# arkworks-rs/snark

Hardware: NVIDIA H100
Metric: groth16_proofs_per_sec (higher is better)
Workload: dtype u32 limbs (255/381-bit modular integers)

## Files before the change

snark_b200/csrc/common.cuh:

```cuda
#pragma once
#include <cuda_runtime.h>

#include <cstdarg>
#include <cstdint>
#include <cstdio>
#include <map>
#include <mutex>
#include <string>
#include <vector>

#include "../../include/b200snark.h"
#include "curves.cuh"

namespace b2s {

struct NttPlan;
struct MsmDedupCache;

struct Ctx {
    int curve = 0;
    int device = 0;
    cudaStream_t stream = nullptr;
    cudaStream_t aux = nullptr;
    cudaEvent_t ev_tail = nullptr, ev_done = nullptr;
// ... 83 lines not shown
            p = nullptr;
            return fail(c, e == cudaErrorMemoryAllocation ? B2S_ERR_OOM : B2S_ERR_CUDA, "cudaMallocAsync(%zu): %s", n,
                        cudaGetErrorString(e));
        }
        return B2S_OK;
    }
    void release() {
        if (p && secret) cudaMemsetAsync(p, 0, bytes, ctx->stream);
        if (p) cudaFreeAsync(p, ctx->stream);
        p = nullptr;
        bytes = 0;
    }
    template <class T>
    T* as() const { return reinterpret_cast<T*>(p); }
};

struct InBuf {
    DevBuf own;
    const void* dptr = nullptr;
    int32_t bind(Ctx* c, const void* src, size_t bytes, int32_t mem) {
        if (mem == B2S_MEM_DEVICE) { dptr = src; return B2S_OK; }
        B2S_TRY(own.alloc(c, bytes));
        if (bytes) B2S_CUDA(c, cudaMemcpyAsync(own.p, src, bytes, cudaMemcpyHostToDevice, c->stream));
        dptr = own.p;
        return B2S_OK;
    }
    template <class T>
    const T* as() const { return reinterpret_cast<const T*>(dptr); }
};

#define B2S_SMEM_ATTR(ctx, kern, bytes) \
    B2S_CUDA(ctx, cudaFuncSetAttribute(kern, cudaFuncAttributeMaxDynamicSharedMemorySize, (int)(bytes)))

struct HostWipe {
    void* p;
    size_t n;
    ~HostWipe() {
        volatile unsigned char* q = reinterpret_cast<volatile unsigned char*>(p);
        for (size_t i = 0; i < n; i++) q[i] = 0;
    }
};

inline unsigned cdiv(uint64_t a, uint64_t b) { return (unsigned)((a + b - 1) / b); }

template <class F>
inline int32_t dispatch_curve(Ctx* c, F&& f) {
    switch (c->curve) {
        case B2S_CURVE_BLS12_381: return f(Bls12_381{});
        case B2S_CURVE_BN254: return f(Bn254{});
        case B2S_CURVE_BLS12_377: return f(Bls12_377{});
    }
    return fail(c, B2S_ERR_INVALID_ARG, "unknown curve id %d", c->curve);
}

struct Sizes {
    size_t fr, fq, g1, g2, g1x, g2x;
    size_t aff(int group) const { return group == 1 ? g1 : g2; }
    size_t xyzz(int group) const { return group == 1 ? g1x : g2x; }
    size_t enc(int group, bool compressed) const { return compressed ? aff(group) / 2 : aff(group); }
};
inline Sizes sizes(const Ctx* c) {
    Sizes s{};
    dispatch_curve(const_cast<Ctx*>(c), [&](auto curve) {
        using C = decltype(curve);
        using Fq = typename C::Fq;
        static_assert(sizeof(typename C::G1Affine) == 2 * sizeof(Fq) && sizeof(typename C::G2Affine) == 4 * sizeof(Fq) &&
                          sizeof(typename C::G1) == 4 * sizeof(Fq) && sizeof(typename C::G2) == 8 * sizeof(Fq),
                      "the ABI points are packed coordinates: 2, 4, 4 and 8 Fq");
        s = {sizeof(typename C::Fr), sizeof(Fq), sizeof(typename C::G1Affine), sizeof(typename C::G2Affine), sizeof(typename C::G1),
             sizeof(typename C::G2)};
        return (int32_t)B2S_OK;
    });
    return s;
}

int32_t ntt_run(Ctx* c, void* data_dev, uint32_t log_n, bool inverse, bool coset);
void ntt_free_plans(Ctx* c);
struct MsmPre { uint32_t c, nwin; uint32_t stride; };
int32_t msm_run(Ctx* c, int group, const void* bases_dev, const void* scalars_dev, uint64_t n, bool scalars_mont,
                void* out_xyzz_dev, void* wins_ext = nullptr, const MsmPre* pre = nullptr);
int32_t msm_run_batch(Ctx* c, int group, const void* bases_dev, const void* scalars_dev, uint64_t n, uint64_t stride, uint32_t K,
                      bool scalars_mont, void* out_xyzz_dev, const MsmPre* pre = nullptr);
uint64_t msm_batch_bytes(Ctx* c, int group, uint64_t n, const MsmPre* pre, uint64_t* max_k);
int32_t msm_precompute(Ctx* c, int group, const void* bases_dev, uint64_t n, void* table_dev, MsmPre* pre);
uint32_t msm_precompute_windows(Ctx* c, uint64_t n, uint32_t* c_out);
int32_t msm_join_tails(Ctx* c);
void msm_dedup_scope_begin(Ctx* c);
void msm_dedup_scope_end(Ctx* c);
int32_t scan_counts(Ctx* c, const uint32_t* counts, uint32_t n, uint32_t L, uint32_t* offsets, uint32_t* task_off);
int32_t fixed_base_run(Ctx* c, int group, const void* scalars_dev, uint64_t n, bool mont, void* out_dev);
int32_t group_sum_to_affine(Ctx* c, int group, const void* xyzz_dev, uint32_t count, void* out_affine_dev);

}
```

snark_b200/csrc/groth16.cu:

```cuda
#include "ec_team.cuh"
#include "r1cs.cuh"

namespace b2s {

template <class Curve>
__global__ void __launch_bounds__(128)
groth16_epilogue_g1_kernel(const Affine<typename Curve::Fq>* consts , const XYZZ<typename Curve::Fq>* sums ,
                           const typename Curve::Fr* rs, uint64_t rs_stride, Affine<typename Curve::Fq>* out_a, Affine<typename Curve::Fq>* out_c) {
    using Fq = typename Curve::Fq;
    using Fr = typename Curve::Fr;
    using P = XYZZ<Fq>;
    __shared__ P sh[3];
    __shared__ P table[3][16];
    const int role = threadIdx.x >> 5;
    const bool lead = (threadIdx.x & 31) == 0;
    sums += blockIdx.x;
    const uint32_t K = gridDim.x;
    rs += blockIdx.x * rs_stride;
    out_a += blockIdx.x;
    out_c += blockIdx.x;
    if (role == 0) {
        P a = sums[2 * K];
        a.add_affine(consts[0]);
        Fr s = rs[1].from_mont();
        P v = team_scalar_mul(a, s.v, Fr::N, table[0]);
        if (lead) sh[0] = v;
    } else if (role == 1) {
        P b = sums[3 * K];
        b.add_affine(consts[1]);
        Fr r = rs[0].from_mont();
        P v = team_scalar_mul(b, r.v, Fr::N, table[1]);
        if (lead) sh[1] = v;
    } else if (role == 2) {
        Fr rsp = (rs[0] * rs[1]).from_mont();
        P v = team_scalar_mul(P::from_affine(consts[2]), rsp.v, Fr::N, table[2]);
        if (lead) sh[2] = v;
    } else {
        P a = sums[2 * K];
        a.add_affine(consts[0]);
        if (lead) *out_a = a.to_affine();
    }
    __syncthreads();
    if (role == 0) {
        P c = sh[0];
        team_add(c, sh[1]);
        team_add(c, sh[2].neg());
        team_add(c, sums[K]);
        team_add(c, sums[0]);
        if (lead) *out_c = c.to_affine();
    }
}

template <class Curve>
__global__ void groth16_epilogue_g2_kernel(const Affine<typename Curve::Fq2>* consts ,
                                           const XYZZ<typename Curve::Fq2>* b2_sum, Affine<typename Curve::Fq2>* out_b) {
    if (threadIdx.x != 0) return;
    XYZZ<typename Curve::Fq2> acc = b2_sum[blockIdx.x];
    acc.add_affine(consts[0]);
    out_b[blockIdx.x] = acc.to_affine();
}

template <class F>
__global__ void sum_shards_kernel(const XYZZ<F>* partials, uint32_t n_shards, uint32_t stride, uint32_t count, XYZZ<F>* sums) {
    const uint32_t j = blockIdx.x * blockDim.x + threadIdx.x;
    if (j >= count) return;
    XYZZ<F> acc = XYZZ<F>::identity();
    for (uint32_t sidx = 0; sidx < n_shards; sidx++) acc.add(partials[sidx * stride + j]);
    sums[j] = acc;
}

int32_t pk_finish(Ctx* c, b2s_pk* pk) {
    const Sizes z = sizes(c);
    const uint64_t n_vars = pk->n_instance + pk->n_witness;
    const char* delta[3] = {nullptr, pk->consts_g1.as<char>() + 2 * z.g1, pk->consts_g2.as<char>() + z.g2};
    for (int w = 0; w < PK_QUERIES; w++) {
        PkQuery& q = pk->q[w];
        const PkQueryInfo& info = PK_QUERY[w];
        const size_t pt = z.aff(info.group);
        q.ext = (info.delta_at >= 0 && q.off + q.len == n_vars) ? 2 : 0;
        char* d = q.pts.as<char>() + q.len * pt;
        B2S_CUDA(c, cudaMemsetAsync(d, 0, 2 * pt, c->stream));
        if (q.ext) B2S_CUDA(c, cudaMemcpyAsync(d + info.delta_at * pt, delta[info.group], pt, cudaMemcpyDeviceToDevice, c->stream));
    }
    const PkQuery& h = pk->q[Q_H];
    {
        const char* env = getenv("B2S_PK_PRECOMP");
        const uint64_t min_n = getenv("B2S_PK_PRECOMP_MIN") ? strtoull(getenv("B2S_PK_PRECOMP_MIN"), nullptr, 10) : (1ull << 18);
        uint32_t cc = 0;
        const uint32_t nw = msm_precompute_windows(c, h.len, &cc);
        size_t free_b = 0, total_b = 0;
        cudaMemGetInfo(&free_b, &total_b);
        const uint64_t need = (uint64_t)nw * h.len * z.g1;
        if (!(env && env[0] == '0') && h.len >= min_n && (uint64_t)nw * h.len < (1ull << 31) && need * 4 < (uint64_t)free_b) {
            B2S_TRY(pk->h_table.alloc(c, need));
            B2S_TRY(msm_precompute(c, 1, h.pts.p, h.len, pk->h_table.p, &pk->h_pre));
        }
    }
    B2S_CUDA(c, cudaStreamSynchronize(c->stream));
    return B2S_OK;
}

int32_t pk_upload(Ctx* c, const b2s_pk_desc* d, int32_t mem, int32_t qap, b2s_pk** out) {
    const Sizes z = sizes(c);
    const uint64_t n_vars = d->n_instance + d->n_witness;
    struct { const void* pts; uint64_t off, len, bound; } src[PK_QUERIES] = {
        {d->a_query, d->a_off, d->a_len, n_vars},
        {d->b_g1_query, d->b1_off, d->b1_len, n_vars},
        {d->b_g2_query, d->b2_off, d->b2_len, n_vars},
        {d->h_query, d->h_off, d->h_len, d->domain_size},
        {d->l_query, d->l_off, d->l_len, d->n_witness}};
    for (const auto& s : src)
        if (s.off + s.len > s.bound) return fail(c, B2S_ERR_MALFORMED_VK, "pk: a query range exceeds the key dimensions");
    if (!d->alpha_g1 || !d->beta_g1 || !d->delta_g1 || !d->beta_g2 || !d->delta_g2)
        return fail(c, B2S_ERR_MALFORMED_VK, "pk: missing group constants");
    if (qap == B2S_QAP_CIRCOM && d->h_off == 0 && d->h_len + 1 == d->domain_size && d->a_len == n_vars && d->b1_len == n_vars &&
        d->b2_len == n_vars && d->l_len == d->n_witness)
        return fail(c, B2S_ERR_MALFORMED_VK, "pk: a full circom key has domain_size = %llu h_query points, not %llu (a libsnark key?)",
                    (unsigned long long)d->domain_size, (unsigned long long)d->h_len);
    b2s_pk* pk = new b2s_pk();
    pk->n_instance = d->n_instance; pk->n_witness = d->n_witness; pk->domain_size = d->domain_size; pk->qap = qap;
    for (int w = 0; w < PK_QUERIES; w++) { pk->q[w].off = src[w].off; pk->q[w].len = src[w].len; }
    const cudaMemcpyKind kind = mem == B2S_MEM_DEVICE ? cudaMemcpyDeviceToDevice : cudaMemcpyHostToDevice;
    auto body = [&]() -> int32_t {
        const size_t g1 = z.g1, g2 = z.g2;
        B2S_TRY(pk->consts_g1.alloc(c, 3 * g1));
        B2S_TRY(pk->consts_g2.alloc(c, 2 * g2));
        char* p1 = pk->consts_g1.as<char>();
        char* p2 = pk->consts_g2.as<char>();
        B2S_CUDA(c, cudaMemcpyAsync(p1, d->alpha_g1, g1, kind, c->stream));
        B2S_CUDA(c, cudaMemcpyAsync(p1 + g1, d->beta_g1, g1, kind, c->stream));
        B2S_CUDA(c, cudaMemcpyAsync(p1 + 2 * g1, d->delta_g1, g1, kind, c->stream));
        B2S_CUDA(c, cudaMemcpyAsync(p2, d->beta_g2, g2, kind, c->stream));
        B2S_CUDA(c, cudaMemcpyAsync(p2 + g2, d->delta_g2, g2, kind, c->stream));
        for (int w = 0; w < PK_QUERIES; w++) {
            const size_t pt = z.aff(PK_QUERY[w].group);
            B2S_TRY(pk->q[w].pts.alloc(c, (src[w].len + 2) * pt));
            if (src[w].len) B2S_CUDA(c, cudaMemcpyAsync(pk->q[w].pts.p, src[w].pts, src[w].len * pt, kind, c->stream));
        }
        return pk_finish(c, pk);
    };
    const int32_t st = body();
    if (st != B2S_OK) { delete pk; return st; }
    *out = pk;
    return B2S_OK;
}

struct ReplicatedH : HSource {
    DevBuf h;
    int32_t get(Ctx* c, const b2s_pk* pk, const b2s_r1cs* m, const void* z_dev, const void** h_for_shard) override {
        B2S_TRY(h.alloc(c, (size_t)32 << m->log_domain));
        B2S_TRY(witness_map_run(c, m, z_dev, h.p, pk->qap));
        *h_for_shard = h.as<char>() + pk->q[Q_H].off * 32;
        return B2S_OK;
    }
};

static int32_t pk_matches(Ctx* c, const b2s_pk* pk, const b2s_r1cs* m) {
    const uint64_t N = 1ull << m->log_domain;
    if (pk->n_instance != m->n_instance || pk->n_witness != m->n_witness || pk->domain_size != N)
        return fail(c, B2S_ERR_ASSIGNMENT_MISSING, "prove: key (%llu,%llu,%llu) does not match matrices (%llu,%llu,%llu)",
                    (unsigned long long)pk->n_instance, (unsigned long long)pk->n_witness, (unsigned long long)pk->domain_size,
                    (unsigned long long)m->n_instance, (unsigned long long)m->n_witness, (unsigned long long)N);
    return B2S_OK;
}

template <class Curve>
static int32_t shard_t(Ctx* c, const b2s_pk* pk, const b2s_r1cs* m, const void* z_inst, const void* z_wit, const void* z_dev,
                       const void* r_host, const void* s_host, void* g1_out, void* g2_out, HSource* hs) {
    using Fr = typename Curve::Fr;
    using P1 = XYZZ<typename Curve::Fq>;
    using P2 = XYZZ<typename Curve::Fq2>;
    B2S_TRY(pk_matches(c, pk, m));
    const uint64_t n_vars = m->n_instance + m->n_witness;
    DevBuf z, tails;
    ReplicatedH replicated;
    if (!hs) hs = &replicated;
    B2S_TRY(z.alloc(c, (n_vars + 2) * sizeof(Fr)));
    B2S_TRY(tails.alloc(c, 4 * 64 * sizeof(P1) + 64 * sizeof(P2)));
// ... 182 lines not shown
```

snark_b200/csrc/msm.cu:

```cuda
#include <algorithm>
#include <array>
#include <cstring>

#include "msm_affine.cuh"

namespace b2s {

__device__ __forceinline__ int32_t recode_digit(uint64_t v, uint32_t off, uint32_t& carry, uint32_t w, uint32_t c, uint32_t nwin) {
    uint32_t d = (uint32_t)((v >> off) & ((1u << c) - 1u)) + carry;
    carry = 0;
    if (w != nwin - 1 && d >= (1u << (c - 1))) {
        carry = 1;
        return (int32_t)d - (int32_t)(1u << c);
    }
    return (int32_t)d;
}

struct DigitIter {
    uint32_t k[8];
    uint32_t carry;
    __device__ __forceinline__ int32_t next(uint32_t w, uint32_t c, uint32_t nwin) {
        const uint32_t bit = w * c;
        const uint32_t word = bit >> 5, off = bit & 31;
        uint64_t v = 0;
// ... 376 lines not shown
            for (uint32_t p = (s + S - bb % S) % S; p < parts; p += S) {
                const uint32_t p0 = lo + p * SORT_SPLIT, p1 = min(hi, p0 + SORT_SPLIT);
                for (uint32_t i = p0 + threadIdx.x; i < p1; i += SORT_THREADS) atomicAdd(&hist[part_fine[i]], 1u);
                __syncthreads();
                for (uint32_t f = threadIdx.x; f < nf; f += SORT_THREADS) {
                    const uint32_t k = hist[f];
                    if (k) cur[f] = offsets[k0 + f] + atomicAdd(&cursor[k0 + f], k);
                    hist[f] = 0;
                }
                __syncthreads();
                for (uint32_t c0 = p0; c0 < p1; c0 += SORT_CHUNK) place_chunk(c0, min(SORT_CHUNK, p1 - c0), nf, part_val, part_fine, sorted, sv, sf, hist, start, cur);
            }
        }
        __syncthreads();
    }
}

struct HeavyPlan { uint32_t split, big, by_ordinal; };
static HeavyPlan heavy_plan(uint32_t G) { return G <= 64 ? HeavyPlan{256u, 512u, 1u} : HeavyPlan{16u, 256u, 0u}; }
static size_t heavy_tmp_slots(const HeavyPlan& hp, uint32_t G, uint64_t max_tasks) {
    return hp.by_ordinal ? (size_t)G * hp.split + 1 : (size_t)(max_tasks / hp.split) + hp.split + 1;
}

template <class F>
__global__ void __launch_bounds__(MSM_RED_THREADS)
msm_reduce_heavy_stage1_kernel(const uint32_t* __restrict__ heavy, const uint32_t* __restrict__ task_off, HeavyPlan hp,
                               const XYZZ<F>* __restrict__ partials, XYZZ<F>* __restrict__ tmp) {
    extern __shared__ uint4 smem_raw[];
    XYZZ<F>* smem = reinterpret_cast<XYZZ<F>*>(smem_raw);
    const uint32_t nitems = heavy[0] * hp.split;
    for (uint32_t it = blockIdx.x; it < nitems; it += gridDim.x) {
        const uint32_t h = it / hp.split, j = it % hp.split;
        const uint32_t g = heavy[1 + h];
        const uint32_t t0 = task_off[g], cnt = task_off[g + 1] - t0;
        if (cnt < hp.big) continue;
        const uint32_t lo = (uint32_t)((uint64_t)cnt * j / hp.split), hi = (uint32_t)((uint64_t)cnt * (j + 1) / hp.split);
        XYZZ<F> s = cta_sum(partials + t0 + lo, hi - lo, smem);
        if (threadIdx.x == 0) st_struct(tmp + (hp.by_ordinal ? h * hp.split : t0 / hp.split) + j, s);
        __syncthreads();
    }
}

template <class F>
__global__ void __launch_bounds__(MSM_RED_THREADS)
msm_reduce_heavy_kernel(const uint32_t* __restrict__ heavy, const uint32_t* __restrict__ task_off, const uint32_t* __restrict__ perm, HeavyPlan hp,
                        const XYZZ<F>* __restrict__ partials, const XYZZ<F>* __restrict__ tmp, XYZZ<F>* __restrict__ bucket_acc) {
    extern __shared__ uint4 smem_raw[];
    XYZZ<F>* smem = reinterpret_cast<XYZZ<F>*>(smem_raw);
    const uint32_t nheavy = heavy[0];
    for (uint32_t h = blockIdx.x; h < nheavy; h += gridDim.x) {
        const uint32_t rk = heavy[1 + h];
        const uint32_t g = perm ? perm[rk] : rk;
        const uint32_t t0 = task_off[rk], cnt = task_off[rk + 1] - t0;
        XYZZ<F> s = cnt < hp.big ? cta_sum(partials + t0, cnt, smem) : cta_sum(tmp + (hp.by_ordinal ? h * hp.split : t0 / hp.split), hp.split, smem);
        if (threadIdx.x == 0) st_struct(bucket_acc + g, s);
        __syncthreads();
    }
}

template <class F>
__global__ void __launch_bounds__(MSM_RED_THREADS)
group_sum_affine_kernel(const XYZZ<F>* __restrict__ pts, uint32_t count, Affine<F>* __restrict__ out) {
    extern __shared__ uint4 smem_raw[];
    XYZZ<F>* smem = reinterpret_cast<XYZZ<F>*>(smem_raw);
    XYZZ<F> s = cta_sum(pts, count, smem);
    if (threadIdx.x == 0) {
        Affine<F> a = s.to_affine();
        st_struct(out, a);
    }
}

int32_t msm_bucket_reduce_g2(Ctx* c, const void* bucket_acc, MsmShape sh, uint32_t seg, void* segs, uint32_t segs_per_win, void* wins) {
    return dispatch_curve(c, [&](auto curve) {
        using F = typename decltype(curve)::Fq2;
        return msm_bucket_reduce_launch<F>(c, "msm_bucket_segments_g2", "msm_window_sum_g2", bucket_acc, sh, seg, segs, segs_per_win, wins);
    });
}

static uint32_t env_u32(const char* name, uint32_t dflt) {
    const char* v = getenv(name);
    return v ? (uint32_t)strtoul(v, nullptr, 10) : dflt;
}

static MsmShape msm_shape(uint64_t n, uint32_t scalar_bits, size_t point_bytes, const MsmPre* pre = nullptr, uint32_t K = 1) {
    MsmShape sh{};
    if (pre) {
        sh.c = pre->c; sh.nwin = pre->nwin; sh.B = 1u << (pre->c - 1); sh.G = K * sh.B; sh.pre_stride = pre->stride;
        const uint64_t t_upper = (uint64_t)K * sh.nwin * n;
        sh.L = (uint32_t)std::max<uint64_t>(64, t_upper >> 18);
        sh.max_tasks = t_upper / sh.L + sh.G + 1;
        return sh;
    }
    auto nwin_of = [&](uint32_t c) {
        uint32_t nw = (scalar_bits + c - 1) / c;
        if (scalar_bits - (nw - 1) * c >= c) nw += 1;
        return nw;
    };
    uint32_t best_c = 5;
    double best = 1e300;
    for (uint32_t c = 5; c <= 20; c++) {
        const uint32_t nw = nwin_of(c);
        const double buckets = (double)nw * (double)(1u << (c - 1));
        if (buckets * (double)point_bytes > 4.0 * 1024 * 1024 * 1024) break;
        const double cost = (double)n * nw + buckets * 4.7;
        if (cost < best) { best = cost; best_c = c; }
    }
    uint32_t c = env_u32("B2S_MSM_C", best_c);
    if (c < 2) c = 2;
    if (c > 24) c = 24;
    sh.c = c;
    sh.nwin = nwin_of(c);
    sh.B = 1u << (c - 1);
    sh.G = K * sh.nwin * sh.B;
    const uint64_t t_upper = (uint64_t)K * sh.nwin * n;
    uint64_t L = t_upper >> 18;
    if (L < 64) L = 64;
    L = env_u32("B2S_MSM_L", (uint32_t)L);
    sh.L = (uint32_t)L;
    sh.max_tasks = t_upper / sh.L + sh.G + 1;
    return sh;
}

struct RoundPlan { uint32_t rounds, L; uint64_t max_tasks; };
template <class F>
static RoundPlan plan_rounds(Ctx* c, uint64_t T, uint32_t G, bool is_g1, uint32_t L_default) {
    RoundPlan rp{0, L_default, T / L_default + G + 1};
    uint32_t ba_auto = 0;
    const uint64_t per_bucket = G ? T / G : 0;
    while ((1ull << ba_auto) < per_bucket) ba_auto++;
    const double min_adds = is_g1 ? 6.0e6 : 2.5e6;
    uint32_t pays = 0;
    while (pays < 16 && (double)(T >> (pays + 1)) > min_adds) pays++;
    ba_auto = std::min(ba_auto, pays);
    rp.rounds = env_u32("B2S_MSM_AFFINE_ROUNDS", ba_auto);
    if (rp.rounds && !getenv("B2S_MSM_AFFINE_ROUNDS")) {
        const uint64_t t0 = std::min<uint64_t>(T, (T + G) / 2 + 1);
        const uint64_t need = t0 * (sizeof(Affine<F>) * 3 / 2 + sizeof(F)) + t0 / 4;
        size_t free_b = (size_t)c->total_mem, total_b = 0;
        uint64_t pool_held = 0;
        if (need * 3 > c->total_mem) {
            cudaMemGetInfo(&free_b, &total_b);
            cudaMemPool_t pool;
            if (cudaDeviceGetDefaultMemPool(&pool, c->device) == cudaSuccess) {
                uint64_t reserved = 0, used = 0;
                cudaMemPoolGetAttribute(pool, cudaMemPoolAttrReservedMemCurrent, &reserved);
                cudaMemPoolGetAttribute(pool, cudaMemPoolAttrUsedMemCurrent, &used);
                pool_held = reserved > used ? reserved - used : 0;
            }
        }
        if (need + ((uint64_t)2 << 30) > (uint64_t)free_b + pool_held) rp.rounds = 0;
    }
    if (rp.rounds && !getenv("B2S_MSM_L")) {
        uint64_t t_after = T;
        for (uint32_t r = 0; r < rp.rounds; r++) t_after = std::min<uint64_t>(t_after, (t_after + G) / 2 + 1);
        rp.L = (uint32_t)std::max<uint64_t>(16, t_after >> 18);
        rp.max_tasks = t_after / rp.L + G + 1;
    }
    return rp;
}

template <class Curve, class F>
static int32_t bucket_sums_t(Ctx* c, const Affine<F>* bases, const uint32_t* sorted, uint32_t* counts, uint32_t* offsets, uint64_t T, uint32_t G,
                             const RoundPlan& rp, XYZZ<F>* bucket_acc) {
    using Pt = XYZZ<F>;
    constexpr bool is_g1 = sizeof(F) == sizeof(typename Curve::Fq);
    MsmShape sh{};
    sh.G = G; sh.L = rp.L; sh.max_tasks = rp.max_tasks;
    const uint32_t ntiles = (G + SCAN_TILE - 1) / SCAN_TILE;
    const uint32_t* no_perm = nullptr;
    DevBuf tiles, tbuf, partials, heavy_tmp;
    B2S_TRY(tiles.alloc(c, (size_t)ntiles * sizeof(Scan3)));
    B2S_TRY(tbuf.alloc(c, ((size_t)2 * G + 3) * sizeof(uint32_t)));
    uint32_t* task_off = tbuf.as<uint32_t>();
    uint32_t* heavy = task_off + G + 1;
    B2S_TRY(partials.alloc(c, (size_t)sh.max_tasks * sizeof(Pt)));
    const HeavyPlan hp = heavy_plan(G);
    B2S_TRY(heavy_tmp.alloc(c, heavy_tmp_slots(hp, G, sh.max_tasks) * sizeof(Pt)));
    const void* acc_bases = bases;
    const uint32_t* acc_sorted = sorted;
    const uint32_t* acc_offsets = offsets;
    const uint32_t* acc_counts = counts;
    DevBuf ba_ints, ba_out[2], ba_prefix, ba_tot, ba_bits;
    if (rp.rounds) {
        B2S_TRY(ba_ints.alloc(c, ((size_t)4 * G + 2) * sizeof(uint32_t)));
        uint32_t* pp_cnt[2] = {ba_ints.as<uint32_t>(), ba_ints.as<uint32_t>() + 2 * G + 1};
        uint32_t* pp_off[2] = {pp_cnt[0] + G, pp_cnt[1] + G};
        const uint32_t* cnt_in = counts;
        uint64_t t_in = T;
        auto round_bound = [&](uint64_t tin) { return std::min<uint64_t>(tin, (tin + G) / 2 + 1); };
        const uint64_t out_bound0 = round_bound(t_in);
        const uint64_t words_bound0 = out_bound0 / 32 + 2;
        const uint64_t tot_bound = (words_bound0 / BA_KMIN + 2) * 32;
        const uint32_t rank_tiles0 = cdiv(words_bound0, BA_SCAN_TILE);
        B2S_TRY(ba_bits.alloc(c, (2 * words_bound0 + rank_tiles0 + 1) * sizeof(uint32_t)));
        uint32_t* bitmap = ba_bits.as<uint32_t>();
        uint32_t* wrank = bitmap + words_bound0;
        uint32_t* rtiles = wrank + words_bound0;
        B2S_TRY(ba_prefix.alloc(c, out_bound0 * sizeof(F)));
        B2S_TRY(ba_tot.alloc(c, 2 * tot_bound * sizeof(F)));
        const uint32_t target_units = 4u * 16u * (uint32_t)c->sm_count;
        DevBuf ba_ctr;
        B2S_TRY(ba_ctr.alloc(c, (size_t)2 * rp.rounds * sizeof(uint32_t)));
        B2S_CUDA(c, cudaMemsetAsync(ba_ctr.p, 0, (size_t)2 * rp.rounds * sizeof(uint32_t), c->stream));
        B2S_TRY(ba_out[1].alloc(c, out_bound0 * sizeof(Affine<F>)));
        if (rp.rounds > 1) B2S_TRY(ba_out[0].alloc(c, round_bound(out_bound0) * sizeof(Affine<F>)));
        const void* prev = nullptr;
        for (uint32_t r = 0; r < rp.rounds; r++) {
            const int nxt = (int)(r & 1u);
            uint32_t* cnt_out = pp_cnt[nxt];
            uint32_t* off_out = pp_off[nxt];
            const uint64_t out_bound = round_bound(t_in);
            const uint32_t n_words = (uint32_t)(out_bound / 32 + 2);
            const uint32_t rank_tiles = cdiv(n_words, BA_SCAN_TILE);
            B2S_LAUNCH(c, msm_ba_halve_kernel, cdiv(G, 256), 256, 0, cnt_in, G, cnt_out);
            B2S_LAUNCH(c, msm_scan_tiles_kernel, ntiles, SCAN_THREADS, 0, (const uint32_t*)cnt_out, no_perm, sh, tiles.as<Scan3>());
            B2S_LAUNCH(c, msm_scan_spine_kernel, 1, 1024, 0, tiles.as<Scan3>(), ntiles, sh, off_out, task_off, heavy);
            B2S_LAUNCH(c, msm_scan_apply_kernel, ntiles, SCAN_THREADS, 0, (const uint32_t*)cnt_out, no_perm, sh, tiles.as<Scan3>(), off_out, task_off, heavy);
            B2S_CUDA(c, cudaMemsetAsync(bitmap, 0, (size_t)n_words * sizeof(uint32_t), c->stream));
            B2S_LAUNCH(c, msm_ba_singles_kernel, cdiv(G, 256), 256, 0, cnt_in, (const uint32_t*)off_out, G, bitmap);
            B2S_LAUNCH(c, msm_ba_rank_tiles_kernel, rank_tiles, BA_SCAN_THREADS, 0, bitmap, n_words, rtiles);
            B2S_LAUNCH(c, msm_ba_rank_spine_kernel, 1, 1024, 0, rtiles, rank_tiles);
            B2S_LAUNCH(c, msm_ba_rank_apply_kernel, rank_tiles, BA_SCAN_THREADS, 0, bitmap, n_words, rtiles, wrank);
            BaRoundArgs ra{};
            ra.first = r == 0;
            ra.bases = bases; ra.sorted = sorted; ra.prev = prev;
            ra.bitmap = bitmap; ra.wrank = wrank; ra.t_out = off_out + G;
            ra.target_units = target_units;
            ra.unit_ctr = ba_ctr.as<uint32_t>() + 2 * r;
            ra.prefix = ba_prefix.p; ra.tot = ba_tot.p; ra.inv_scratch = ba_tot.as<F>() + tot_bound; ra.out = ba_out[nxt ^ 1].p;
            if (is_g1) B2S_TRY(msm_ba_round_g1(c, ra));
            else B2S_TRY(msm_ba_round_g2(c, ra));
            prev = ba_out[nxt ^ 1].p;
            t_in = out_bound;
            cnt_in = cnt_out;
        }
        acc_bases = prev;
        acc_sorted = nullptr;
        acc_offsets = pp_off[(rp.rounds - 1) & 1u];
        acc_counts = pp_cnt[(rp.rounds - 1) & 1u];
    } else {
        B2S_LAUNCH(c, msm_scan_tiles_kernel, ntiles, SCAN_THREADS, 0, counts, no_perm, sh, tiles.as<Scan3>());
        B2S_LAUNCH(c, msm_scan_spine_kernel, 1, 1024, 0, tiles.as<Scan3>(), ntiles, sh, offsets, task_off, heavy);
        B2S_LAUNCH(c, msm_scan_apply_kernel, ntiles, SCAN_THREADS, 0, counts, no_perm, sh, tiles.as<Scan3>(), offsets, task_off, heavy);
    }
    const uint32_t* perm = nullptr;
    DevBuf perm_buf;
    if (!rp.rounds && G >= 1024) {
        B2S_TRY(perm_buf.alloc(c, ((size_t)G + 2 * SIZE_BINS) * sizeof(uint32_t)));
        uint32_t* pm = perm_buf.as<uint32_t>();
        uint32_t* hist = pm + G;
        uint32_t* binoff = hist + SIZE_BINS;
        uint32_t* none = nullptr;
        B2S_CUDA(c, cudaMemsetAsync(hist, 0, SIZE_BINS * sizeof(uint32_t), c->stream));
        B2S_LAUNCH(c, msm_size_hist_kernel, cdiv(G, 256), 256, 0, acc_counts, G, hist);
        B2S_LAUNCH(c, msm_size_scan_kernel, 1, 1024, 0, hist, binoff);
        B2S_LAUNCH(c, msm_size_scatter_kernel, cdiv(G, 256), 256, 0, acc_counts, G, binoff, hist, pm);
        B2S_LAUNCH(c, msm_scan_tiles_kernel, ntiles, SCAN_THREADS, 0, acc_counts, (const uint32_t*)pm, sh, tiles.as<Scan3>());
        B2S_LAUNCH(c, msm_scan_spine_kernel, 1, 1024, 0, tiles.as<Scan3>(), ntiles, sh, none, task_off, heavy);
        B2S_LAUNCH(c, msm_scan_apply_kernel, ntiles, SCAN_THREADS, 0, acc_counts, (const uint32_t*)pm, sh, tiles.as<Scan3>(), none, task_off, heavy);
        perm = pm;
    }
    if (is_g1) B2S_TRY(msm_accumulate_g1(c, acc_bases, acc_sorted, acc_offsets, task_off, perm, sh, bucket_acc, partials.p));
    else B2S_TRY(msm_accumulate_g2(c, acc_bases, acc_sorted, acc_offsets, task_off, perm, sh, bucket_acc, partials.p));
    const size_t red_smem = (size_t)MSM_RED_THREADS * sizeof(Pt);
    B2S_SMEM_ATTR(c, msm_reduce_heavy_kernel<F>, red_smem);
    B2S_SMEM_ATTR(c, msm_reduce_heavy_stage1_kernel<F>, red_smem);
    B2S_LAUNCH(c, msm_reduce_heavy_stage1_kernel<F>, 4 * c->sm_count, MSM_RED_THREADS, red_smem, heavy, task_off, hp,
               partials.as<Pt>(), heavy_tmp.as<Pt>());
    B2S_LAUNCH(c, msm_reduce_heavy_kernel<F>, 2 * c->sm_count, MSM_RED_THREADS, red_smem, heavy, task_off, perm, hp,
               partials.as<Pt>(), heavy_tmp.as<Pt>(), bucket_acc);
    return B2S_OK;
}

template <class Curve, class F>
static int32_t msm_core_t(Ctx* c, const Affine<F>* bases, const typename Curve::Fr* scalars, const uint32_t* index_map, uint64_t n, bool mont,
                          XYZZ<F>* out, void* wins_ext, bool* used_aux = nullptr, const MsmPre* pre = nullptr, uint32_t K = 1, uint64_t stride = 0) {
    using Fr = typename Curve::Fr;
    using Pt = XYZZ<F>;
    constexpr bool is_g1 = sizeof(F) == sizeof(typename Curve::Fq);
    if (n == 0) {
        B2S_CUDA(c, cudaMemsetAsync(out, 0, K * sizeof(Pt), c->stream));
        return B2S_OK;
    }
    MsmShape sh = msm_shape(n, Curve::FrP::BITS, sizeof(Pt), pre, K);
    if ((uint64_t)K * sh.nwin * n >= (1ull << 32) || (uint64_t)K * sh.nwin * sh.B >= (1ull << 32))
        return fail(c, B2S_ERR_INVALID_ARG, "msm: vectors * n * windows exceeds 2^32");
    if (pre && (uint64_t)pre->nwin * pre->stride >= (1ull << 31)) return fail(c, B2S_ERR_INVALID_ARG, "msm: precomputed table exceeds 2^31 points");
    const RoundPlan rp = plan_rounds<F>(c, (uint64_t)K * sh.nwin * n, sh.G, is_g1, sh.L);
    sh.L = rp.L; sh.max_tasks = rp.max_tasks;
    const uint32_t MSM_SEG = sh.B >= (1u << 16) ? 32u : 16u;
    const uint32_t ntiles = (sh.G + SCAN_TILE - 1) / SCAN_TILE;
    DevBuf ibuf, sorted, bucket_acc, segs, wins, tiles;
    B2S_TRY(tiles.alloc(c, (size_t)ntiles * sizeof(Scan3)));
    const size_t ints = (size_t)5 * sh.G + 3;
    B2S_TRY(ibuf.alloc(c, ints * sizeof(uint32_t)));
    uint32_t* counts = ibuf.as<uint32_t>();
    uint32_t* cursor = counts + sh.G;
    uint32_t* offsets = cursor + sh.G;
    uint32_t* task_off = offsets + sh.G + 1;
    uint32_t* heavy = task_off + sh.G + 1;
    B2S_CUDA(c, cudaMemsetAsync(counts, 0, (size_t)2 * sh.G * sizeof(uint32_t), c->stream));
    const uint64_t T = (uint64_t)K * sh.nwin * n;
    B2S_TRY(sorted.alloc(c, (size_t)T * sizeof(uint32_t)));
    B2S_TRY(bucket_acc.alloc(c, (size_t)sh.G * sizeof(Pt)));
    B2S_CUDA(c, cudaMemsetAsync(bucket_acc.p, 0, (size_t)sh.G * sizeof(Pt), c->stream));
    const uint32_t segs_per_win = (sh.B + MSM_SEG - 1) / MSM_SEG;
    MsmShape sh_red = sh;
    sh_red.nwin = K * (pre ? 1u : sh.nwin);
    B2S_TRY(segs.alloc(c, (size_t)segs_per_win * sh_red.nwin * sizeof(Pt)));
    if (sh.nwin > 64 || K > 1) wins_ext = nullptr;
    if (!wins_ext) B2S_TRY(wins.alloc(c, (size_t)std::max(sh.nwin, sh_red.nwin) * sizeof(Pt)));
    Pt* wins_p = wins_ext ? reinterpret_cast<Pt*>(wins_ext) : wins.as<Pt>();

    B2S_LAUNCH(c, msm_count_kernel<Fr>, dim3(cdiv(n, 256), K), 256, 0, scalars, n, stride, mont, sh, counts);
    const uint32_t* no_perm = nullptr;
    B2S_LAUNCH(c, msm_scan_tiles_kernel, ntiles, SCAN_THREADS, 0, counts, no_perm, sh, tiles.as<Scan3>());
    B2S_LAUNCH(c, msm_scan_spine_kernel, 1, 1024, 0, tiles.as<Scan3>(), ntiles, sh, offsets, task_off, heavy);
    B2S_LAUNCH(c, msm_scan_apply_kernel, ntiles, SCAN_THREADS, 0, counts, no_perm, sh, tiles.as<Scan3>(), offsets, task_off, heavy);
    {
        const uint32_t fine_bits = sort_fine_bits(sh.c), nbins = sh.G >> fine_bits, nbw = sh.B >> fine_bits;
        DevBuf part;
        B2S_TRY(part.alloc(c, (size_t)T * (sizeof(uint32_t) + sizeof(uint16_t)) + (size_t)nbins * sizeof(uint32_t)));
        uint32_t* part_val = part.as<uint32_t>();
        uint32_t* bin_cursor = part_val + T;
        uint16_t* part_fine = reinterpret_cast<uint16_t*>(bin_cursor + nbins);
        B2S_CUDA(c, cudaMemsetAsync(bin_cursor, 0, (size_t)nbins * sizeof(uint32_t), c->stream));
        B2S_SMEM_ATTR(c, msm_partition_kernel<Fr>, partition_smem(nbw));
        B2S_SMEM_ATTR(c, msm_place_kernel, place_smem(fine_bits));
        B2S_LAUNCH(c, msm_partition_kernel<Fr>, dim3(cdiv(n, SORT_TILE), K), SORT_THREADS, partition_smem(nbw), scalars, index_map, n, stride, mont, sh,
                   fine_bits, (const uint32_t*)offsets, bin_cursor, part_val, part_fine);
        B2S_LAUNCH(c, msm_place_kernel, nbins + c->sm_count, SORT_THREADS, place_smem(fine_bits), (const uint32_t*)offsets, nbins, fine_bits,
                   (const uint32_t*)part_val, (const uint16_t*)part_fine, cursor, sorted.as<uint32_t>());
    }
    B2S_TRY((bucket_sums_t<Curve, F>(c, bases, sorted.as<uint32_t>(), counts, offsets, T, sh.G, rp, bucket_acc.as<Pt>())));
    if (is_g1) B2S_TRY(msm_bucket_reduce_g1(c, bucket_acc.p, sh_red, MSM_SEG, segs.p, segs_per_win, wins_p));
    else B2S_TRY(msm_bucket_reduce_g2(c, bucket_acc.p, sh_red, MSM_SEG, segs.p, segs_per_win, wins_p));
    if (!wins_ext) {
        B2S_TRY(msm_horner(c, c->stream, is_g1 ? 1 : 2, wins_p, sh_red, K, out));
    } else {
        B2S_CUDA(c, cudaEventRecord(c->ev_tail, c->stream));
        B2S_CUDA(c, cudaStreamWaitEvent(c->aux, c->ev_tail, 0));
        B2S_TRY(msm_horner(c, c->aux, is_g1 ? 1 : 2, wins_p, sh_red, K, out));
        c->aux_pending = true;
        if (used_aux) *used_aux = true;
    }
    return B2S_OK;
}

static constexpr uint32_t DEDUP_SAMPLES = 1024, DEDUP_MAX = 8;
struct DedupCand { uint32_t v[DEDUP_MAX][8]; uint32_t k; };

template <class Fr>
__global__ void msm_sample_kernel(const Fr* __restrict__ scalars, uint64_t n, uint64_t stride, Fr* __restrict__ out) {
    const uint32_t t = blockIdx.x * blockDim.x + threadIdx.x;
    if (t >= DEDUP_SAMPLES) return;
    const uint64_t i = (uint64_t)t * stride;
    if (i < n) st_struct(out + t, ld_struct(scalars + i));
}
template <class Fr>
__device__ __forceinline__ uint32_t dedup_gid(const Fr& s, const DedupCand& cd) {
    uint32_t nz = 0;
#pragma unroll
    for (int j = 0; j < 8; j++) nz |= s.v[j];
    if (nz == 0) return DEDUP_MAX + 1;
    for (uint32_t k = 0; k < cd.k; k++) {
        uint32_t d = 0;
#pragma unroll
        for (int j = 0; j < 8; j++) d |= s.v[j] ^ cd.v[k][j];
        if (d == 0) return k;
    }
    return DEDUP_MAX;
}
template <class Fr, int PASS>
// ... 196 lines not shown
        }
        B2S_LAUNCH_SN(c, ts, is_g1 ? "msm_tiny_products_g1" : "msm_tiny_products_g2", (msm_tiny_products_kernel<Curve, F>), count, 32, 0, bases,
                      (const uint32_t*)rest_idx.as<uint32_t>(), (const Fr*)rest_scal.as<Fr>(), (uint32_t)n_rest, (const Pt*)hsums, cd, mont, prods);
        B2S_LAUNCH_SN(c, ts, is_g1 ? "msm_tiny_sum_g1" : "msm_tiny_sum_g2", msm_tiny_sum_kernel<F>, 1, 32, 0, (const Pt*)prods, count, out);
        if (on_aux) c->aux_pending = true;
        return B2S_OK;
    }
    bool used_aux = false;
    B2S_TRY((msm_core_t<Curve, F>(c, bases, rest_scal.as<Fr>(), rest_idx.as<uint32_t>(), n_rest, mont, out, wins_ext, &used_aux, pre)));
    cudaStream_t fs = used_aux ? c->aux : c->stream;
    const size_t fin_smem = ((size_t)DEDUP_MAX * 16 + DEDUP_MAX) * sizeof(Pt);
    B2S_SMEM_ATTR(c, (msm_heavy_finish_kernel<Curve, F>), fin_smem);
    B2S_LAUNCH_SN(c, fs, is_g1 ? "msm_heavy_finish_g1" : "msm_heavy_finish_g2", (msm_heavy_finish_kernel<Curve, F>), 1, 32 * DEDUP_MAX, fin_smem,
                  (const Pt*)hsums, cd, mont, out);
    return B2S_OK;
}

int32_t scan_counts(Ctx* c, const uint32_t* counts, uint32_t n, uint32_t L, uint32_t* offsets, uint32_t* task_off) {
    MsmShape sh{};
    sh.G = n;
    sh.L = L;
    const uint32_t ntiles = (n + SCAN_TILE - 1) / SCAN_TILE;
    DevBuf tiles, heavy;
    B2S_TRY(tiles.alloc(c, (size_t)ntiles * sizeof(Scan3)));
    B2S_TRY(heavy.alloc(c, ((size_t)n + 1) * sizeof(uint32_t)));
    const uint32_t* no_perm = nullptr;
    B2S_LAUNCH(c, msm_scan_tiles_kernel, ntiles, SCAN_THREADS, 0, counts, no_perm, sh, tiles.as<Scan3>());
    B2S_LAUNCH(c, msm_scan_spine_kernel, 1, 1024, 0, tiles.as<Scan3>(), ntiles, sh, offsets, task_off, heavy.as<uint32_t>());
    B2S_LAUNCH(c, msm_scan_apply_kernel, ntiles, SCAN_THREADS, 0, counts, no_perm, sh, tiles.as<Scan3>(), offsets, task_off, heavy.as<uint32_t>());
    return B2S_OK;
}

int32_t msm_join_tails(Ctx* c) {
    if (!c->aux_pending) return B2S_OK;
    B2S_CUDA(c, cudaEventRecord(c->ev_done, c->aux));
    B2S_CUDA(c, cudaStreamWaitEvent(c->stream, c->ev_done, 0));
    c->aux_pending = false;
    return B2S_OK;
}

int32_t msm_run(Ctx* c, int group, const void* bases_dev, const void* scalars_dev, uint64_t n, bool scalars_mont,
                void* out_xyzz_dev, void* wins_ext, const MsmPre* pre) {
    return dispatch_curve(c, [&](auto curve) {
        using C = decltype(curve);
        if (group == 1) return msm_run_t<C, typename C::Fq>(c, bases_dev, scalars_dev, n, scalars_mont, out_xyzz_dev, wins_ext, pre);
        return msm_run_t<C, typename C::Fq2>(c, bases_dev, scalars_dev, n, scalars_mont, out_xyzz_dev, wins_ext, pre);
    });
}

int32_t msm_run_batch(Ctx* c, int group, const void* bases_dev, const void* scalars_dev, uint64_t n, uint64_t stride, uint32_t K,
                      bool scalars_mont, void* out_xyzz_dev, const MsmPre* pre) {
    if (n >= (1ull << 31)) return fail(c, B2S_ERR_INVALID_ARG, "msm: n = %llu exceeds 2^31 - 1", (unsigned long long)n);
    return dispatch_curve(c, [&](auto curve) {
        using C = decltype(curve);
        const auto* s = reinterpret_cast<const typename C::Fr*>(scalars_dev);
        if (group == 1) {
            using F = typename C::Fq;
            return msm_core_t<C, F>(c, reinterpret_cast<const Affine<F>*>(bases_dev), s, nullptr, n, scalars_mont, reinterpret_cast<XYZZ<F>*>(out_xyzz_dev),
                                    nullptr, nullptr, pre, K, stride);
        }
        using F = typename C::Fq2;
        return msm_core_t<C, F>(c, reinterpret_cast<const Affine<F>*>(bases_dev), s, nullptr, n, scalars_mont, reinterpret_cast<XYZZ<F>*>(out_xyzz_dev),
                                nullptr, nullptr, pre, K, stride);
    });
}

static uint32_t fr_bits(Ctx* c) {
    uint32_t bits = 0;
    dispatch_curve(c, [&](auto curve) { bits = decltype(curve)::FrP::BITS; return (int32_t)B2S_OK; });
    return bits;
}

uint64_t msm_batch_bytes(Ctx* c, int group, uint64_t n, const MsmPre* pre, uint64_t* max_k) {
    const Sizes z = sizes(c);
    const uint32_t bits = fr_bits(c);
    const size_t pt = z.xyzz(group);
    const MsmShape sh = msm_shape(std::max<uint64_t>(n, 1), bits, pt, pre);
    const uint64_t T = (uint64_t)sh.nwin * n, G = sh.G;
    *max_k = std::max<uint64_t>(1, std::min(((1ull << 32) - 1) / std::max<uint64_t>(T, 1), ((1ull << 32) - 1) / G));
    const uint64_t fe = z.aff(group) / 2;
    return G * (pt + 5 * sizeof(uint32_t)) + T * (sizeof(uint32_t) * 2 + sizeof(uint16_t)) + (T / 16 + G) * pt + T * (3 * fe + fe) / 2;
}

template <class F>
__global__ void __launch_bounds__(128) msm_precompute_kernel(const Affine<F>* __restrict__ bases, uint64_t n, uint32_t c, uint32_t nwin, Affine<F>* __restrict__ table) {
    const uint64_t i = (uint64_t)blockIdx.x * blockDim.x + threadIdx.x;
    if (i >= n) return;
    const Affine<F> p = ld_struct(bases + i);
    st_struct(table + i, p);
    XYZZ<F> acc = XYZZ<F>::from_affine(p);
    for (uint32_t w = 1; w < nwin; w++) {
        for (uint32_t k = 0; k < c; k++) acc = acc.dbl();
        const Affine<F> q = acc.to_affine();
        st_struct(table + (uint64_t)w * n + i, q);
        acc = XYZZ<F>::from_affine(q);
    }
}

uint32_t msm_precompute_windows(Ctx* c, uint64_t n, uint32_t* c_out) {
    (void)n;
    const uint32_t bits = fr_bits(c);
    const uint32_t cc = env_u32("B2S_MSM_PRE_C", 20);
    uint32_t nw = (bits + cc - 1) / cc;
    if (bits - (nw - 1) * cc >= cc) nw += 1;
    if (c_out) *c_out = cc;
    return nw;
}

int32_t msm_precompute(Ctx* c, int group, const void* bases_dev, uint64_t n, void* table_dev, MsmPre* pre) {
    uint32_t cc = 0;
    const uint32_t nw = msm_precompute_windows(c, n, &cc);
    if ((uint64_t)nw * n >= (1ull << 31)) return fail(c, B2S_ERR_INVALID_ARG, "msm_precompute: table of %u x %llu points exceeds 2^31", nw, (unsigned long long)n);
    pre->c = cc; pre->nwin = nw; pre->stride = (uint32_t)n;
    if (n == 0) return B2S_OK;
    return dispatch_curve(c, [&](auto curve) {
        using C = decltype(curve);
        if (group == 1)
            B2S_LAUNCH_N(c, "msm_precompute_g1", msm_precompute_kernel<typename C::Fq>, cdiv(n, 128), 128, 0, reinterpret_cast<const Affine<typename C::Fq>*>(bases_dev), n,
                         cc, nw, reinterpret_cast<Affine<typename C::Fq>*>(table_dev));
        else
            B2S_LAUNCH_N(c, "msm_precompute_g2", msm_precompute_kernel<typename C::Fq2>, cdiv(n, 128), 128, 0, reinterpret_cast<const Affine<typename C::Fq2>*>(bases_dev),
                         n, cc, nw, reinterpret_cast<Affine<typename C::Fq2>*>(table_dev));
        return (int32_t)B2S_OK;
    });
}

template <class Curve, class F>
static int32_t group_sum_t(Ctx* c, const void* xyzz_dev, uint32_t count, void* out_affine_dev) {
    const size_t red_smem = (size_t)MSM_RED_THREADS * sizeof(XYZZ<F>);
    B2S_CUDA(c, cudaFuncSetAttribute(group_sum_affine_kernel<F>, cudaFuncAttributeMaxDynamicSharedMemorySize, (int)red_smem));
    B2S_LAUNCH(c, group_sum_affine_kernel<F>, 1, MSM_RED_THREADS, red_smem, reinterpret_cast<const XYZZ<F>*>(xyzz_dev),
               count, reinterpret_cast<Affine<F>*>(out_affine_dev));
    return B2S_OK;
}

int32_t group_sum_to_affine(Ctx* c, int group, const void* xyzz_dev, uint32_t count, void* out_affine_dev) {
    return dispatch_curve(c, [&](auto curve) {
        using C = decltype(curve);
        if (group == 1) return group_sum_t<C, typename C::Fq>(c, xyzz_dev, count, out_affine_dev);
        return group_sum_t<C, typename C::Fq2>(c, xyzz_dev, count, out_affine_dev);
    });
}

}
```

Measured before the change: 4.871.

## Slice affine bucket rounds to fit memory budget and refine H-table precompute check

When the batch-affine round scratch does not fit in free memory, the bucket accumulation is now split into bucket-range slices. Each slice fits the budget, so affine rounds can stay enabled instead of being turned off. The slice boundaries come from a binary search on the bucket offsets, which needs a host synchronisation and readback. The H-query precompute decision now uses a computed MSM working set plus idle pool memory instead of a crude free-memory ratio, which may enable the precomputed table more often.

```diff
diff --git a/snark_b200/csrc/common.cuh b/snark_b200/csrc/common.cuh
--- a/snark_b200/csrc/common.cuh
+++ b/snark_b200/csrc/common.cuh
@@ -189,6 +189,8 @@
 int32_t msm_run_batch(Ctx* c, int group, const void* bases_dev, const void* scalars_dev, uint64_t n, uint64_t stride, uint32_t K,
                       bool scalars_mont, void* out_xyzz_dev, const MsmPre* pre = nullptr);
 uint64_t msm_batch_bytes(Ctx* c, int group, uint64_t n, const MsmPre* pre, uint64_t* max_k);
+void msm_working_set(Ctx* c, int group, uint64_t n, const MsmPre* pre, uint64_t* sort_bytes, uint64_t* round_bytes);
+uint64_t pool_idle_bytes(Ctx* c);
 int32_t msm_precompute(Ctx* c, int group, const void* bases_dev, uint64_t n, void* table_dev, MsmPre* pre);
 uint32_t msm_precompute_windows(Ctx* c, uint64_t n, uint32_t* c_out);
 int32_t msm_join_tails(Ctx* c);
diff --git a/snark_b200/csrc/groth16.cu b/snark_b200/csrc/groth16.cu
--- a/snark_b200/csrc/groth16.cu
+++ b/snark_b200/csrc/groth16.cu
@@ -88,12 +88,23 @@
         const uint64_t min_n = getenv("B2S_PK_PRECOMP_MIN") ? strtoull(getenv("B2S_PK_PRECOMP_MIN"), nullptr, 10) : (1ull << 18);
         uint32_t cc = 0;
         const uint32_t nw = msm_precompute_windows(c, h.len, &cc);
-        size_t free_b = 0, total_b = 0;
-        cudaMemGetInfo(&free_b, &total_b);
         const uint64_t need = (uint64_t)nw * h.len * z.g1;
-        if (!(env && env[0] == '0') && h.len >= min_n && (uint64_t)nw * h.len < (1ull << 31) && need * 4 < (uint64_t)free_b) {
-            B2S_TRY(pk->h_table.alloc(c, need));
-            B2S_TRY(msm_precompute(c, 1, h.pts.p, h.len, pk->h_table.p, &pk->h_pre));
+        if (!(env && env[0] == '0') && h.len >= min_n && (uint64_t)nw * h.len < (1ull << 31)) {
+            const MsmPre h_shape{cc, nw, (uint32_t)h.len};
+            uint64_t sort_max = 0, rounds_h = 0;
+            for (int w = 0; w < PK_QUERIES; w++) {
+                uint64_t sort_b = 0, round_b = 0;
+                msm_working_set(c, PK_QUERY[w].group, pk->q[w].len + pk->q[w].ext, w == Q_H ? &h_shape : nullptr, &sort_b, &round_b);
+                sort_max = std::max(sort_max, sort_b);
+                if (w == Q_H) rounds_h = round_b;
+            }
+            const uint64_t working = 7 * pk->domain_size * z.fr + sort_max + rounds_h + ((uint64_t)2 << 30);
+            size_t free_b = 0, total_b = 0;
+            cudaMemGetInfo(&free_b, &total_b);
+            if (need + working <= (uint64_t)free_b + pool_idle_bytes(c)) {
+                B2S_TRY(pk->h_table.alloc(c, need));
+                B2S_TRY(msm_precompute(c, 1, h.pts.p, h.len, pk->h_table.p, &pk->h_pre));
+            }
         }
     }
     B2S_CUDA(c, cudaStreamSynchronize(c->stream));
diff --git a/snark_b200/csrc/msm.cu b/snark_b200/csrc/msm.cu
--- a/snark_b200/csrc/msm.cu
+++ b/snark_b200/csrc/msm.cu
@@ -482,6 +482,15 @@
     return v ? (uint32_t)strtoul(v, nullptr, 10) : dflt;
 }
 
+uint64_t pool_idle_bytes(Ctx* c) {
+    cudaMemPool_t pool;
+    if (cudaDeviceGetDefaultMemPool(&pool, c->device) != cudaSuccess) return 0;
+    uint64_t reserved = 0, used = 0;
+    cudaMemPoolGetAttribute(pool, cudaMemPoolAttrReservedMemCurrent, &reserved);
+    cudaMemPoolGetAttribute(pool, cudaMemPoolAttrUsedMemCurrent, &used);
+    return reserved > used ? reserved - used : 0;
+}
+
 static MsmShape msm_shape(uint64_t n, uint32_t scalar_bits, size_t point_bytes, const MsmPre* pre = nullptr, uint32_t K = 1) {
     MsmShape sh{};
     if (pre) {
@@ -521,47 +530,68 @@
     return sh;
 }
 
-struct RoundPlan { uint32_t rounds, L; uint64_t max_tasks; };
-template <class F>
-static RoundPlan plan_rounds(Ctx* c, uint64_t T, uint32_t G, bool is_g1, uint32_t L_default) {
-    RoundPlan rp{0, L_default, T / L_default + G + 1};
-    uint32_t ba_auto = 0;
-    const uint64_t per_bucket = G ? T / G : 0;
-    while ((1ull << ba_auto) < per_bucket) ba_auto++;
-    const double min_adds = is_g1 ? 6.0e6 : 2.5e6;
-    uint32_t pays = 0;
-    while (pays < 16 && (double)(T >> (pays + 1)) > min_adds) pays++;
-    ba_auto = std::min(ba_auto, pays);
-    rp.rounds = env_u32("B2S_MSM_AFFINE_ROUNDS", ba_auto);
-    if (rp.rounds && !getenv("B2S_MSM_AFFINE_ROUNDS")) {
-        const uint64_t t0 = std::min<uint64_t>(T, (T + G) / 2 + 1);
-        const uint64_t need = t0 * (sizeof(Affine<F>) * 3 / 2 + sizeof(F)) + t0 / 4;
-        size_t free_b = (size_t)c->total_mem, total_b = 0;
-        uint64_t pool_held = 0;
-        if (need * 3 > c->total_mem) {
-            cudaMemGetInfo(&free_b, &total_b);
-            cudaMemPool_t pool;
-            if (cudaDeviceGetDefaultMemPool(&pool, c->device) == cudaSuccess) {
-                uint64_t reserved = 0, used = 0;
-                cudaMemPoolGetAttribute(pool, cudaMemPoolAttrReservedMemCurrent, &reserved);
-                cudaMemPoolGetAttribute(pool, cudaMemPoolAttrUsedMemCurrent, &used);
-                pool_held = reserved > used ? reserved - used : 0;
-            }
-        }
-        if (need + ((uint64_t)2 << 30) > (uint64_t)free_b + pool_held) rp.rounds = 0;
-    }
+struct RoundPlan { uint32_t rounds, L; uint64_t max_tasks; uint64_t slice_entries; uint32_t L_plain; };
+
+static uint64_t round_scratch_bytes(uint64_t T, uint64_t G, size_t aff, size_t xyzz) {
+    const uint64_t t0 = std::min<uint64_t>(T, (T + G) / 2 + 1);
+    return t0 * (aff * 3 / 2 + aff / 2) + t0 / 4 + (G + std::min<uint64_t>(t0 / 16 + 1, 1u << 18)) * xyzz;
+}
+
+static void plan_tasks(RoundPlan& rp, uint64_t T, uint32_t G) {
+    rp.L = rp.L_plain;
+    rp.max_tasks = T / rp.L + G + 1;
     if (rp.rounds && !getenv("B2S_MSM_L")) {
         uint64_t t_after = T;
         for (uint32_t r = 0; r < rp.rounds; r++) t_after = std::min<uint64_t>(t_after, (t_after + G) / 2 + 1);
         rp.L = (uint32_t)std::max<uint64_t>(16, t_after >> 18);
         rp.max_tasks = t_after / rp.L + G + 1;
     }
+}
+
+template <class F>
+static RoundPlan plan_rounds(Ctx* c, uint64_t T, uint32_t G, bool is_g1, uint32_t L_default, uint64_t held = 0) {
+    RoundPlan rp{0, L_default, 0, T, L_default};
+    uint32_t ba_auto = 0;
+    const uint64_t per_bucket = G ? T / G : 0;
+    while ((1ull << ba_auto) < per_bucket) ba_auto++;
+    const double min_adds = is_g1 ? 6.0e6 : 2.5e6;
+    auto pays = [&](uint64_t t) {
+        uint32_t p = 0;
+        while (p < 16 && (double)(t >> (p + 1)) > min_adds) p++;
+        return std::min(ba_auto, p);
+    };
+    const bool forced = getenv("B2S_MSM_AFFINE_ROUNDS") != nullptr;
+    rp.rounds = forced ? env_u32("B2S_MSM_AFFINE_ROUNDS", 0) : pays(T);
+    const char* budget_env = getenv("B2S_MSM_ROUND_BUDGET");
+    if (rp.rounds && (budget_env || !forced)) {
+        const uint64_t need = round_scratch_bytes(T, G, sizeof(Affine<F>), sizeof(XYZZ<F>));
+        uint64_t budget = 0;
+        if (budget_env) {
+            budget = strtoull(budget_env, nullptr, 10);
+        } else {
+            size_t free_b = (size_t)c->total_mem, total_b = 0;
+            uint64_t pool_held = 0;
+            if ((need + held) * 3 > c->total_mem) {
+                cudaMemGetInfo(&free_b, &total_b);
+                pool_held = pool_idle_bytes(c);
+            }
+            const uint64_t avail = (uint64_t)free_b + pool_held, reserve = held + ((uint64_t)2 << 30);
+            budget = avail > reserve ? avail - reserve : 0;
+        }
+        if (need > budget) {
+            rp.slice_entries = (uint64_t)((double)T * ((double)budget / (double)need));
+            if (!forced && rp.slice_entries) rp.rounds = pays(T / ((T + rp.slice_entries - 1) / rp.slice_entries));
+            if (rp.slice_entries < 2 * std::max<uint64_t>(per_bucket, 1)) rp.rounds = 0;
+            if (!rp.rounds) rp.slice_entries = T;
+        }
+    }
+    plan_tasks(rp, T, G);
     return rp;
 }
 
 template <class Curve, class F>
-static int32_t bucket_sums_t(Ctx* c, const Affine<F>* bases, const uint32_t* sorted, uint32_t* counts, uint32_t* offsets, uint64_t T, uint32_t G,
-                             const RoundPlan& rp, XYZZ<F>* bucket_acc) {
+static int32_t bucket_slice_t(Ctx* c, const Affine<F>* bases, const uint32_t* sorted, uint32_t* counts, uint32_t* offsets, uint64_t T, uint32_t G,
+                              const RoundPlan& rp, XYZZ<F>* bucket_acc) {
     using Pt = XYZZ<F>;
     constexpr bool is_g1 = sizeof(F) == sizeof(typename Curve::Fq);
     MsmShape sh{};
@@ -672,6 +702,53 @@
     return B2S_OK;
 }
 
+__global__ void msm_slice_bounds_kernel(const uint32_t* __restrict__ offsets, uint32_t G, uint64_t T, uint32_t S, uint2* __restrict__ bounds) {
+    const uint32_t k = blockIdx.x * blockDim.x + threadIdx.x;
+    if (k > S) return;
+    const uint64_t e = T * k / S;
+    uint32_t lo = 0, hi = G;
+    while (lo < hi) {
+        const uint32_t mid = (lo + hi) >> 1;
+        if (offsets[mid] < e) lo = mid + 1; else hi = mid;
+    }
+    bounds[k] = make_uint2(lo, offsets[lo]);
+}
+
+template <class Curve, class F>
+static int32_t bucket_sums_t(Ctx* c, const Affine<F>* bases, const uint32_t* sorted, uint32_t* counts, uint32_t* offsets, uint64_t T, uint32_t G,
+                             const RoundPlan& rp, XYZZ<F>* bucket_acc) {
+    if (!rp.rounds || rp.slice_entries >= T) return bucket_slice_t<Curve, F>(c, bases, sorted, counts, offsets, T, G, rp, bucket_acc);
+    std::vector<uint2> hb;
+    uint32_t S = (uint32_t)std::min<uint64_t>(G, (T + rp.slice_entries - 1) / rp.slice_entries);
+    for (int tries = 0;; tries++) {
+        DevBuf db;
+        B2S_TRY(db.alloc(c, ((size_t)S + 1) * sizeof(uint2)));
+        B2S_LAUNCH(c, msm_slice_bounds_kernel, cdiv(S + 1, 256), 256, 0, (const uint32_t*)offsets, G, T, S, db.as<uint2>());
+        hb.resize((size_t)S + 1);
+        B2S_CUDA(c, cudaMemcpyAsync(hb.data(), db.p, hb.size() * sizeof(uint2), cudaMemcpyDeviceToHost, c->stream));
+        B2S_CUDA(c, cudaStreamSynchronize(c->stream));
+        uint64_t largest = 0;
+        for (uint32_t k = 0; k < S; k++) largest = std::max<uint64_t>(largest, hb[k + 1].y - hb[k].y);
+        if (largest <= rp.slice_entries) break;
+        if (tries == 3 || S >= G) {
+            RoundPlan plain = rp;
+            plain.rounds = 0;
+            plain.slice_entries = T;
+            plan_tasks(plain, T, G);
+            return bucket_slice_t<Curve, F>(c, bases, sorted, counts, offsets, T, G, plain, bucket_acc);
+        }
+        S = std::min<uint32_t>(G, 2 * S);
+    }
+    for (uint32_t k = 0; k < S; k++) {
+        const uint32_t g0 = hb[k].x, g1 = hb[k + 1].x, e0 = hb[k].y, e1 = hb[k + 1].y;
+        if (e1 == e0) continue;
+        RoundPlan sp = rp;
+        plan_tasks(sp, e1 - e0, g1 - g0);
+        B2S_TRY((bucket_slice_t<Curve, F>(c, bases, sorted + e0, counts + g0, offsets + g0, e1 - e0, g1 - g0, sp, bucket_acc + g0)));
+    }
+    return B2S_OK;
+}
+
 template <class Curve, class F>
 static int32_t msm_core_t(Ctx* c, const Affine<F>* bases, const typename Curve::Fr* scalars, const uint32_t* index_map, uint64_t n, bool mont,
                           XYZZ<F>* out, void* wins_ext, bool* used_aux = nullptr, const MsmPre* pre = nullptr, uint32_t K = 1, uint64_t stride = 0) {
@@ -686,9 +763,11 @@
     if ((uint64_t)K * sh.nwin * n >= (1ull << 32) || (uint64_t)K * sh.nwin * sh.B >= (1ull << 32))
         return fail(c, B2S_ERR_INVALID_ARG, "msm: vectors * n * windows exceeds 2^32");
     if (pre && (uint64_t)pre->nwin * pre->stride >= (1ull << 31)) return fail(c, B2S_ERR_INVALID_ARG, "msm: precomputed table exceeds 2^31 points");
-    const RoundPlan rp = plan_rounds<F>(c, (uint64_t)K * sh.nwin * n, sh.G, is_g1, sh.L);
+    const uint32_t MSM_SEG = sh.B >= (1u << 16) ? 32u : 16u;
+    const uint64_t held = (uint64_t)sh.G * (5 * sizeof(uint32_t) + sizeof(Pt)) + (uint64_t)K * sh.nwin * n * sizeof(uint32_t) +
+                          (uint64_t)K * (pre ? 1u : sh.nwin) * ((sh.B + MSM_SEG - 1) / MSM_SEG) * sizeof(Pt);
+    const RoundPlan rp = plan_rounds<F>(c, (uint64_t)K * sh.nwin * n, sh.G, is_g1, sh.L, held);
     sh.L = rp.L; sh.max_tasks = rp.max_tasks;
-    const uint32_t MSM_SEG = sh.B >= (1u << 16) ? 32u : 16u;
     const uint32_t ntiles = (sh.G + SCAN_TILE - 1) / SCAN_TILE;
     DevBuf ibuf, sorted, bucket_acc, segs, wins, tiles;
     B2S_TRY(tiles.alloc(c, (size_t)ntiles * sizeof(Scan3)));
@@ -1051,6 +1130,16 @@
     return G * (pt + 5 * sizeof(uint32_t)) + T * (sizeof(uint32_t) * 2 + sizeof(uint16_t)) + (T / 16 + G) * pt + T * (3 * fe + fe) / 2;
 }
 
+void msm_working_set(Ctx* c, int group, uint64_t n, const MsmPre* pre, uint64_t* sort_bytes, uint64_t* round_bytes) {
+    const Sizes z = sizes(c);
+    const size_t pt = z.xyzz(group);
+    const MsmShape sh = msm_shape(std::max<uint64_t>(n, 1), fr_bits(c), pt, pre);
+    const uint64_t T = (uint64_t)sh.nwin * n, G = sh.G;
+    const uint64_t segs = (uint64_t)(pre ? 1u : sh.nwin) * (sh.B / 16 + 1);
+    *sort_bytes = G * (5 * sizeof(uint32_t) + pt) + segs * pt + T * (2 * sizeof(uint32_t) + sizeof(uint16_t));
+    *round_bytes = round_scratch_bytes(T, G, z.aff(group), pt);
+}
+
 template <class F>
 __global__ void __launch_bounds__(128) msm_precompute_kernel(const Affine<F>* __restrict__ bases, uint64_t n, uint32_t c, uint32_t nwin, Affine<F>* __restrict__ table) {
     const uint64_t i = (uint64_t)blockIdx.x * blockDim.x + threadIdx.x;
```

Result: faster. 5.187, median of 6 (+6.5%).
